# VITA-Group/CV_A-FAN

Measured on AMD Instinct MI355X. Metric: images/sec (whole node) A-FAN K=5 train step, ResNet-18/CIFAR-10, higher is better.
Workload: dtype bf16; 1 GPU; resnet18 CIFAR-10-shape A-FAN K=5 bf16, batch 256/GPU, perturb_idx 6, internal layout nhwc, 1xMI355X per rank (BASELINE configs[1]); global_batch=256, parallelism=dp1, hipgraph=True, in_launch_batchnorm=True

## Files before the change

cv_a-fan_amd/csrc/afan_conv_stem.hip:

```cpp
#include "afan_conv_stem.h"
#include <stdlib.h>

using namespace afan;

namespace afan_stem {
namespace {

typedef __bf16 bf16x8 __attribute__((ext_vector_type(8)));
typedef float f32x16 __attribute__((ext_vector_type(16)));
typedef uint32_t u32x4 __attribute__((ext_vector_type(4)));

constexpr int THREADS = 256;
constexpr int WAVES = THREADS / 64;
constexpr int ROWE = 104;
constexpr uint32_t OOB = 0x80000000u;

__device__ __forceinline__ int slot_elem(int s) {
    const int d = s >> 1, r = d / 5, m = d - 5 * r, e = 2 * m + (s & 1);
    return (d < 15 && e < 9) ? r * 9 + e : -1;
}

__device__ __forceinline__ void stage_rows(const __amdgpu_buffer_rsrc_t xr, uint16_t (*in)[ROWE], int n, int h, int w0, int H,
                                           int W, int lane) {
#pragma unroll
    for (int r = 0; r < 3; ++r) {
        const int hh = h + r - 1;
#pragma unroll
        for (int j = 0; j < 2; ++j) {
            const int i = lane + 64 * j;
            const int px = i / 3, c = i - 3 * px, ww = w0 - 1 + px;
            const bool ok = i < 102 && hh >= 0 && hh < H && ww >= 0 && ww < W;
            const uint32_t off = ok ? (uint32_t)((((n * H + hh) * W + ww) * 3 + c) * 2) : OOB;
            const uint16_t v = (uint16_t)__builtin_amdgcn_raw_buffer_load_b16(xr, (int)off, 0, 0);
            if (i < ROWE) in[r][i] = v;
        }
    }
}

__device__ __forceinline__ void window_frags(const uint16_t (*in)[ROWE], int col, int half, bf16x8& f0, bf16x8& f1) {
    uint32_t D[16];
#pragma unroll
    for (int r = 0; r < 3; ++r) {
        uint32_t e[9];
#pragma unroll
        for (int k = 0; k < 9; ++k) e[k] = in[r][3 * col + k];
        D[5 * r + 0] = e[0] | (e[1] << 16);
        D[5 * r + 1] = e[2] | (e[3] << 16);
        D[5 * r + 2] = e[4] | (e[5] << 16);
        D[5 * r + 3] = e[6] | (e[7] << 16);
        D[5 * r + 4] = e[8];
    }
    D[15] = 0;
    u32x4 a, b;
#pragma unroll
    for (int q = 0; q < 4; ++q) {
        a[q] = half ? D[4 + q] : D[q];
        b[q] = half ? D[12 + q] : D[8 + q];
    }
    f0 = __builtin_bit_cast(bf16x8, a);
    f1 = __builtin_bit_cast(bf16x8, b);
}

struct FwdP {
    const uint16_t* x; const uint16_t* w; uint16_t* y;
    int N, H, W, Co;
    double* acc; int acc_ns; const float* shift;
    const float* aff; int aff_relu;
};

template <int CG, bool AFF>
__global__ __launch_bounds__(THREADS) void stem_fwd_kernel(const FwdP p) {
    constexpr int LDO = CG * 32 + 8;
    __shared__ __attribute__((aligned(16))) uint16_t in_s[WAVES][3][ROWE];
    __shared__ __attribute__((aligned(16))) uint16_t out_s[WAVES][32][LDO];
    __shared__ float red[WAVES][2][CG * 32];
    const int tid = threadIdx.x, lane = tid & 63, wave = tid >> 6, half = lane >> 5, col = lane & 31;
    const int H = p.H, W = p.W, Co = p.Co;
    const __amdgpu_buffer_rsrc_t xr = __builtin_amdgcn_make_buffer_rsrc(
        const_cast<uint16_t*>(p.x), 0, (int)((int64_t)p.N * H * W * 3 * 2), 0x00020000);

    bf16x8 wf[CG][2];
#pragma unroll
    for (int cg = 0; cg < CG; ++cg) {
        const int co = cg * 32 + col;
#pragma unroll
        for (int ks = 0; ks < 2; ++ks) {
            u32x4 v;
#pragma unroll
            for (int q = 0; q < 4; ++q) {
                const int s = 16 * ks + 8 * half + 2 * q;
                const int e0 = slot_elem(s), e1 = slot_elem(s + 1);
                const uint32_t lo = (co < Co && e0 >= 0) ? p.w[co * 27 + e0] : 0u;
                const uint32_t hi = (co < Co && e1 >= 0) ? p.w[co * 27 + e1] : 0u;
                v[q] = lo | (hi << 16);
            }
            wf[cg][ks] = __builtin_bit_cast(bf16x8, v);
        }
    }

    const int ppr = Co >> 3;
    const int pieces = 32 * ppr;
    const int chunk = lane & (ppr - 1);
    const bool want_stats = !AFF && p.acc != nullptr;
    float s1[8], s2[8], sh[8], al[8], be[8];
#pragma unroll
    for (int j = 0; j < 8; ++j) {
        s1[j] = s2[j] = 0.f;
        sh[j] = (want_stats && p.shift) ? p.shift[chunk * 8 + j] : 0.f;
        if constexpr (AFF) {
            al[j] = p.aff[2 * Co + chunk * 8 + j];
            be[j] = p.aff[3 * Co + chunk * 8 + j];
        }
    }

    const int tpr = W >> 5;
    const int tiles = p.N * H * tpr;
    for (int t = blockIdx.x * WAVES + wave; t < tiles; t += gridDim.x * WAVES) {
        const int rowidx = t / tpr, w0 = (t - rowidx * tpr) << 5;
        const int n = rowidx / H, h = rowidx - n * H;
        stage_rows(xr, in_s[wave], n, h, w0, H, W, lane);
        __builtin_amdgcn_wave_barrier();
        bf16x8 f0, f1;
        window_frags(in_s[wave], col, half, f0, f1);
#pragma unroll
        for (int cg = 0; cg < CG; ++cg) {
            f32x16 acc;
#pragma unroll
            for (int r = 0; r < 16; ++r) acc[r] = 0.f;
            acc = __builtin_amdgcn_mfma_f32_32x32x16_bf16(wf[cg][0], f0, acc, 0, 0, 0);
            acc = __builtin_amdgcn_mfma_f32_32x32x16_bf16(wf[cg][1], f1, acc, 0, 0, 0);
#pragma unroll
            for (int g = 0; g < 4; ++g) {
                u16x4 v;
#pragma unroll
                for (int e = 0; e < 4; ++e) v[e] = f2bf(acc[4 * g + e]);
                *reinterpret_cast<u16x4*>(&out_s[wave][col][cg * 32 + 8 * g + 4 * half]) = v;
            }
        }
        __builtin_amdgcn_wave_barrier();
        uint16_t* ytile = p.y + ((int64_t)rowidx * W + w0) * Co;
        for (int q = lane; q < pieces; q += 64) {
            const int px = q / ppr;
            u16x8 v = *reinterpret_cast<const u16x8*>(&out_s[wave][px][chunk * 8]);
            if constexpr (AFF) {
#pragma unroll
                for (int j = 0; j < 8; ++j) {
                    float t = fmaf(bf2f(v[j]), al[j], be[j]);
                    if (p.aff_relu) t = (t > 0.f) ? t : ((t != t) ? t : 0.f);
                    v[j] = f2bf(t);
                }
            }
            *reinterpret_cast<u16x8*>(ytile + px * Co + chunk * 8) = v;
            if (want_stats) {
#pragma unroll
                for (int j = 0; j < 8; ++j) {
                    const float f = bf2f(v[j]) - sh[j];
                    s1[j] += f;
                    s2[j] += f * f;
                }
            }
        }
        __builtin_amdgcn_wave_barrier();
    }

    if (want_stats) {
        for (int o = ppr; o < 64; o <<= 1)
#pragma unroll
            for (int j = 0; j < 8; ++j) {
                s1[j] += __shfl_xor(s1[j], o, 64);
                s2[j] += __shfl_xor(s2[j], o, 64);
            }
        if (lane < ppr) {
#pragma unroll
            for (int j = 0; j < 8; ++j) {
                red[wave][0][lane * 8 + j] = s1[j];
                red[wave][1][lane * 8 + j] = s2[j];
            }
        }
        __syncthreads();
        if (tid < Co) {
            float a = 0.f, b = 0.f;
#pragma unroll
            for (int w = 0; w < WAVES; ++w) {
                a += red[w][0][tid];
                b += red[w][1][tid];
            }
            double* dst = p.acc + (int64_t)(blockIdx.x & (p.acc_ns - 1)) * 2 * Co;
            unsafeAtomicAdd(dst + tid, (double)a);
            unsafeAtomicAdd(dst + Co + tid, (double)b);
            if (blockIdx.x == 0) reinterpret_cast<float*>(p.acc + (int64_t)2 * p.acc_ns * Co)[tid] = p.shift ? p.shift[tid] : 0.f;
        }
    }
}

struct WgradP {
    const uint16_t* x; const uint16_t* dy; float* slab;
    int N, H, W, Co;
};

template <int CG>
__global__ __launch_bounds__(THREADS) void stem_wgrad_kernel(const WgradP p) {
    constexpr int LDY = CG * 32 + 8;
    __shared__ __attribute__((aligned(16))) uint16_t in_s[WAVES][3][ROWE];
    __shared__ __attribute__((aligned(16))) uint16_t dy_s[WAVES][32][LDY];
    __shared__ float part[WAVES][CG * 32][33];
    const int tid = threadIdx.x, lane = tid & 63, wave = tid >> 6, half = lane >> 5, col = lane & 31;
    const int H = p.H, W = p.W, Co = p.Co;
    const __amdgpu_buffer_rsrc_t xr = __builtin_amdgcn_make_buffer_rsrc(
        const_cast<uint16_t*>(p.x), 0, (int)((int64_t)p.N * H * W * 3 * 2), 0x00020000);
    const int se = slot_elem(col);
    const int sr = se >= 0 ? se / 9 : 0, sofs = se >= 0 ? se - 9 * sr : 0;

    f32x16 acc[CG];
#pragma unroll
    for (int cg = 0; cg < CG; ++cg)
#pragma unroll
        for (int r = 0; r < 16; ++r) acc[cg][r] = 0.f;

    const int ppr = Co >> 3, pieces = 32 * ppr, chunk = lane & (ppr - 1);
    const int tpr = W >> 5;
    const int tiles = p.N * H * tpr;
    for (int t = blockIdx.x * WAVES + wave; t < tiles; t += gridDim.x * WAVES) {
        const int rowidx = t / tpr, w0 = (t - rowidx * tpr) << 5;
        const int n = rowidx / H, h = rowidx - n * H;
        stage_rows(xr, in_s[wave], n, h, w0, H, W, lane);
        const uint16_t* dyt = p.dy + ((int64_t)rowidx * W + w0) * Co;
        for (int q = lane; q < pieces; q += 64) {
            const int px = q / ppr;
            *reinterpret_cast<u16x8*>(&dy_s[wave][px][chunk * 8]) = *reinterpret_cast<const u16x8*>(dyt + px * Co + chunk * 8);
        }
        if (CG * 32 > Co)
            for (int q = lane; q < 32 * (CG * 32 - Co); q += 64) dy_s[wave][q / (CG * 32 - Co)][Co + q % (CG * 32 - Co)] = 0;
        __builtin_amdgcn_wave_barrier();
#pragma unroll
        for (int ks = 0; ks < 2; ++ks) {
            const int p0 = 16 * ks + 8 * half;
            u32x4 b;
#pragma unroll
            for (int q = 0; q < 4; ++q) {
                const uint32_t lo = se >= 0 ? in_s[wave][sr][3 * (p0 + 2 * q) + sofs] : 0u;
                const uint32_t hi = se >= 0 ? in_s[wave][sr][3 * (p0 + 2 * q + 1) + sofs] : 0u;
                b[q] = lo | (hi << 16);
            }
            const bf16x8 fb = __builtin_bit_cast(bf16x8, b);
#pragma unroll
            for (int cg = 0; cg < CG; ++cg) {
                u32x4 a;
#pragma unroll
                for (int q = 0; q < 4; ++q) {
                    const uint32_t lo = dy_s[wave][p0 + 2 * q][cg * 32 + col];
                    const uint32_t hi = dy_s[wave][p0 + 2 * q + 1][cg * 32 + col];
                    a[q] = lo | (hi << 16);
                }
                acc[cg] = __builtin_amdgcn_mfma_f32_32x32x16_bf16(__builtin_bit_cast(bf16x8, a), fb, acc[cg], 0, 0, 0);
            }
        }
        __builtin_amdgcn_wave_barrier();
    }
#pragma unroll
    for (int cg = 0; cg < CG; ++cg)
#pragma unroll
        for (int g = 0; g < 4; ++g)
#pragma unroll
            for (int e = 0; e < 4; ++e) part[wave][cg * 32 + 8 * g + 4 * half + e][col] = acc[cg][4 * g + e];
    __syncthreads();
    float* slab = p.slab + (int64_t)blockIdx.x * Co * 27;
    for (int i = tid; i < Co * 32; i += THREADS) {
        const int co = i >> 5, s = i & 31, el = slot_elem(s);
        if (el >= 0) {
            float v = 0.f;
#pragma unroll
            for (int w = 0; w < WAVES; ++w) v += part[w][co][s];
            slab[co * 27 + el] = v;
        }
    }
}

__global__ __launch_bounds__(1024) void stem_wgrad_reduce_kernel(const float* __restrict__ slab, float* __restrict__ grad,
                                                                 int total, int S, int accumulate) {
    __shared__ float red[16][64];
    const int e = threadIdx.x & 63, q = threadIdx.x >> 6;
    const int i = blockIdx.x * 64 + e;
    float v = 0.f;
    if (i < total)
        for (int s = q; s < S; s += 16) v += slab[(int64_t)s * total + i];
    red[q][e] = v;
    __syncthreads();
    if (q == 0 && i < total) {
        float sum = 0.f;
#pragma unroll
        for (int k = 0; k < 16; ++k) sum += red[k][e];
        grad[i] = accumulate ? grad[i] + sum : sum;
    }
}

int wgrad_slabs(int64_t tiles) {
    int64_t g = (tiles + WAVES - 1) / WAVES;
    if (g > 256) g = 256;
    return (int)(g < 1 ? 1 : g);
}

}

bool eligible(int64_t n, int64_t h, int64_t w, int64_t ci, int64_t co, int k, int stride) {
    static const bool on = [] { const char* v = getenv("AFAN_CONV_STEM"); return !v || atoi(v) != 0; }();
    if (!on || ci != 3 || k != 3 || stride != 1) return false;
    if (!(co == 16 || co == 32 || co == 64) || w % 32 != 0 || n <= 0 || h <= 0) return false;
    return n * h * w * co * 2 <= 0x7fffffffLL;
}

static int64_t fwd_grid(int64_t tiles) {
    int64_t g = (tiles + WAVES - 1) / WAVES;
    static const int64_t cap = [] { const char* v = getenv("AFAN_STEM_WGS"); return v ? (int64_t)atoi(v) : (int64_t)1024; }();
    if (g > cap) g = cap;
    return g;
}

int fwd_aff_launch(const void* x, const void* w, void* y, int64_t n, int64_t h, int64_t wd, int64_t co, const float* coefs, int relu,
                   hipStream_t st) {
    FwdP p{(const uint16_t*)x, (const uint16_t*)w, (uint16_t*)y, (int)n, (int)h, (int)wd, (int)co, nullptr, 0, nullptr, coefs, relu ? 1 : 0};
    const int64_t g = fwd_grid(n * h * (wd / 32));
    if (co > 32) stem_fwd_kernel<2, true><<<(unsigned)g, THREADS, 0, st>>>(p);
    else stem_fwd_kernel<1, true><<<(unsigned)g, THREADS, 0, st>>>(p);
    AFAN_LAUNCH_CHECK();
    AFAN_TRACE_LAUNCH("stem_fwd_aff<%d>", co > 32 ? 2 : 1);
    return AFAN_OK;
}

int fwd_launch(const void* x, const void* w, void* y, int64_t n, int64_t h, int64_t wd, int64_t co, double* acc, int acc_ns,
               const float* shift, hipStream_t st) {
    FwdP p{(const uint16_t*)x, (const uint16_t*)w, (uint16_t*)y, (int)n, (int)h, (int)wd, (int)co, acc, acc_ns, shift, nullptr, 0};
    const int64_t tiles = n * h * (wd / 32);
    const int64_t g = fwd_grid(tiles);
    if (co > 32) stem_fwd_kernel<2, false><<<(unsigned)g, THREADS, 0, st>>>(p);
    else stem_fwd_kernel<1, false><<<(unsigned)g, THREADS, 0, st>>>(p);
    AFAN_LAUNCH_CHECK();
    AFAN_TRACE_LAUNCH("stem_fwd<%d>", co > 32 ? 2 : 1);
    return AFAN_OK;
}

int64_t wgrad_workspace_floats(int64_t n, int64_t h, int64_t w, int64_t co) {
    return (int64_t)wgrad_slabs(n * h * (w / 32)) * co * 27;
}

int wgrad_launch(const void* x, const void* dy, float* grad, int64_t n, int64_t h, int64_t wd, int64_t co, float* ws,
                 int accumulate, hipStream_t st) {
    WgradP p{(const uint16_t*)x, (const uint16_t*)dy, ws, (int)n, (int)h, (int)wd, (int)co};
    const int S = wgrad_slabs(n * h * (wd / 32));
    if (co > 32) stem_wgrad_kernel<2><<<S, THREADS, 0, st>>>(p);
    else stem_wgrad_kernel<1><<<S, THREADS, 0, st>>>(p);
    AFAN_LAUNCH_CHECK();
    AFAN_TRACE_LAUNCH("stem_wgrad<%d>", co > 32 ? 2 : 1);
    const int total = (int)co * 27;
    stem_wgrad_reduce_kernel<<<(total + 63) / 64, 1024, 0, st>>>(ws, grad, total, S, accumulate);
    AFAN_LAUNCH_CHECK();
    return AFAN_OK;
}

}
```

Measured before the change: 34650 images/sec.

## Prefetch next tile's input and dy into registers in stem conv kernels

```diff
diff --git a/cv_a-fan_amd/csrc/afan_conv_stem.hip b/cv_a-fan_amd/csrc/afan_conv_stem.hip
--- a/cv_a-fan_amd/csrc/afan_conv_stem.hip
+++ b/cv_a-fan_amd/csrc/afan_conv_stem.hip
@@ -20,8 +20,8 @@
     return (d < 15 && e < 9) ? r * 9 + e : -1;
 }
 
-__device__ __forceinline__ void stage_rows(const __amdgpu_buffer_rsrc_t xr, uint16_t (*in)[ROWE], int n, int h, int w0, int H,
-                                           int W, int lane) {
+__device__ __forceinline__ void request_rows(const __amdgpu_buffer_rsrc_t xr, uint16_t (&v)[6], int n, int h, int w0, int H, int W,
+                                             int lane) {
 #pragma unroll
     for (int r = 0; r < 3; ++r) {
         const int hh = h + r - 1;
@@ -31,10 +31,19 @@
             const int px = i / 3, c = i - 3 * px, ww = w0 - 1 + px;
             const bool ok = i < 102 && hh >= 0 && hh < H && ww >= 0 && ww < W;
             const uint32_t off = ok ? (uint32_t)((((n * H + hh) * W + ww) * 3 + c) * 2) : OOB;
-            const uint16_t v = (uint16_t)__builtin_amdgcn_raw_buffer_load_b16(xr, (int)off, 0, 0);
-            if (i < ROWE) in[r][i] = v;
-        }
-    }
+            v[2 * r + j] = (uint16_t)__builtin_amdgcn_raw_buffer_load_b16(xr, (int)off, 0, 0);
+        }
+    }
+}
+
+__device__ __forceinline__ void write_rows(uint16_t (*in)[ROWE], const uint16_t (&v)[6], int lane) {
+#pragma unroll
+    for (int r = 0; r < 3; ++r)
+#pragma unroll
+        for (int j = 0; j < 2; ++j) {
+            const int i = lane + 64 * j;
+            if (i < ROWE) in[r][i] = v[2 * r + j];
+        }
 }
 
 __device__ __forceinline__ void window_frags(const uint16_t (*in)[ROWE], int col, int half, bf16x8& f0, bf16x8& f1) {
@@ -115,11 +124,20 @@
 
     const int tpr = W >> 5;
     const int tiles = p.N * H * tpr;
-    for (int t = blockIdx.x * WAVES + wave; t < tiles; t += gridDim.x * WAVES) {
+    const int tstep = gridDim.x * WAVES;
+    uint16_t rows[6];
+    auto request = [&](int tt) {
+        const int rowidx = tt / tpr, w0 = (tt - rowidx * tpr) << 5;
+        const int n = rowidx / H, h = rowidx - n * H;
+        request_rows(xr, rows, n, h, w0, H, W, lane);
+    };
+    int t = blockIdx.x * WAVES + wave;
+    if (t < tiles) request(t);
+    for (; t < tiles; t += tstep) {
         const int rowidx = t / tpr, w0 = (t - rowidx * tpr) << 5;
-        const int n = rowidx / H, h = rowidx - n * H;
-        stage_rows(xr, in_s[wave], n, h, w0, H, W, lane);
-        __builtin_amdgcn_wave_barrier();
+        write_rows(in_s[wave], rows, lane);
+        __builtin_amdgcn_wave_barrier();
+        if (t + tstep < tiles) request(t + tstep);
         bf16x8 f0, f1;
         window_frags(in_s[wave], col, half, f0, f1);
 #pragma unroll
@@ -220,18 +238,37 @@
     const int ppr = Co >> 3, pieces = 32 * ppr, chunk = lane & (ppr - 1);
     const int tpr = W >> 5;
     const int tiles = p.N * H * tpr;
-    for (int t = blockIdx.x * WAVES + wave; t < tiles; t += gridDim.x * WAVES) {
-        const int rowidx = t / tpr, w0 = (t - rowidx * tpr) << 5;
+    if (CG * 32 > Co)
+        for (int q = lane; q < 32 * (CG * 32 - Co); q += 64) dy_s[wave][q / (CG * 32 - Co)][Co + q % (CG * 32 - Co)] = 0;
+    const __amdgpu_buffer_rsrc_t dyr = __builtin_amdgcn_make_buffer_rsrc(
+        const_cast<uint16_t*>(p.dy), 0, (int)((int64_t)p.N * H * W * Co * 2), 0x00020000);
+    const int lp = __builtin_ctz(ppr);
+    const int tstep = gridDim.x * WAVES;
+    uint16_t rows[6];
+    u16x8 dyv[CG * 2];
+    auto request = [&](int tt) {
+        const int rowidx = tt / tpr, w0 = (tt - rowidx * tpr) << 5;
         const int n = rowidx / H, h = rowidx - n * H;
-        stage_rows(xr, in_s[wave], n, h, w0, H, W, lane);
-        const uint16_t* dyt = p.dy + ((int64_t)rowidx * W + w0) * Co;
-        for (int q = lane; q < pieces; q += 64) {
-            const int px = q / ppr;
-            *reinterpret_cast<u16x8*>(&dy_s[wave][px][chunk * 8]) = *reinterpret_cast<const u16x8*>(dyt + px * Co + chunk * 8);
-        }
-        if (CG * 32 > Co)
-            for (int q = lane; q < 32 * (CG * 32 - Co); q += 64) dy_s[wave][q / (CG * 32 - Co)][Co + q % (CG * 32 - Co)] = 0;
-        __builtin_amdgcn_wave_barrier();
+        request_rows(xr, rows, n, h, w0, H, W, lane);
+        const int base = (rowidx * W + w0) * Co + chunk * 8;
+#pragma unroll
+        for (int i = 0; i < CG * 2; ++i) {
+            const int q = lane + 64 * i;
+            const uint32_t off = q < pieces ? (uint32_t)((base + (q >> lp) * Co) * 2) : OOB;
+            dyv[i] = __builtin_bit_cast(u16x8, __builtin_amdgcn_raw_buffer_load_b128(dyr, (int)off, 0, 0));
+        }
+    };
+    int t = blockIdx.x * WAVES + wave;
+    if (t < tiles) request(t);
+    for (; t < tiles; t += tstep) {
+        write_rows(in_s[wave], rows, lane);
+#pragma unroll
+        for (int i = 0; i < CG * 2; ++i) {
+            const int q = lane + 64 * i;
+            if (q < pieces) *reinterpret_cast<u16x8*>(&dy_s[wave][q >> lp][chunk * 8]) = dyv[i];
+        }
+        __builtin_amdgcn_wave_barrier();
+        if (t + tstep < tiles) request(t + tstep);
 #pragma unroll
         for (int ks = 0; ks < 2; ++ks) {
             const int p0 = 16 * ks + 8 * half;
```

Result: no change. 34630 images/sec (-0.1%).
